# randyjhc/vit-colmap

Hardware: AMD Instinct MI355X
Metric: images/sec extracted + pair-matches/sec (N×D brute-force NN) (higher is better)
Workload: dtype bf16 (ViT) / u8+i32 (matcher); 1 GPU; configs[1]+configs[2]: DINOv2 ViT-S/14 extract of 50 640x480 images (512 keypoints, 384-D uint8 descriptors) then exhaustive mutual-NN + ratio matching of all pairs among the extracted images; images_total=50, images_rank0=50, num_keypoints=512, descriptor_dim=384, parallelism=images+pairs sharded x1

## Files before the change

vit_colmap_amd/csrc/attention.hip:

```cpp
#include <hip/hip_runtime.h>
#include <stdint.h>

#include "../../include/vitcolmap_hip.h"
#include "common.h"
#include "device.h"

namespace {

typedef __bf16 v8bf __attribute__((ext_vector_type(8)));
typedef __bf16 v4bf __attribute__((ext_vector_type(4)));
typedef __bf16 v2bf __attribute__((ext_vector_type(2)));
typedef short v4s __attribute__((ext_vector_type(4)));
typedef float v16f __attribute__((ext_vector_type(16)));

constexpr int kHD = 64;
constexpr int kWavesA = 4;
constexpr int kQW = 32;
constexpr int kQB = kWavesA * kQW;
constexpr int kKV = 64;
constexpr int kTileBytes = kKV * kHD * 2;

__device__ inline uint32_t k_off(int key, int slot) { return (uint32_t)key * 128u + (uint32_t)((slot ^ (key & 7)) << 4); }
__device__ inline uint32_t v_off(int key, int byte_in_row) {
  return (uint32_t)key * 128u + ((uint32_t)byte_in_row ^ (uint32_t)(((key >> 1) & 1) << 6));
}

constexpr float kLazyTh = 6.0f;
template <int QT, bool LAZY>
__global__ __launch_bounds__(256, (QT == 1 ? 3 : 2)) void attention_kernel(const __bf16* __restrict__ qkv,
                                                                           __bf16* __restrict__ out, int N, int H,
                                                                           float scale_log2e, int unit0, int nqb) {
  __shared__ __attribute__((aligned(16))) uint8_t lds[3][2][kTileBytes];
  const int tid = threadIdx.x, lane = tid & 63, wave = tid >> 6;
  const int r = lane & 31, hh = lane >> 5;
  const int unit = unit0 + (int)blockIdx.x;
  const int bh = unit / nqb, b = bh / H, h = bh - b * H;
  const int q_base = (unit - bh * nqb) * (kQB * QT);
  if (q_base >= N) return;
  const int q_row0 = q_base + wave * (kQW * QT) + r;
  const size_t tok_stride = (size_t)3 * H * kHD;
  const __bf16* base = qkv + (size_t)b * N * tok_stride + (size_t)h * kHD;

  v8bf qf[QT][4];
#pragma unroll
  for (int qt = 0; qt < QT; ++qt) {
    const __bf16* qp = base + (size_t)min(q_row0 + 32 * qt, N - 1) * tok_stride;
#pragma unroll
    for (int ks = 0; ks < 4; ++ks) qf[qt][ks] = *(const v8bf*)(qp + 16 * ks + 8 * hh);
  }
  __builtin_amdgcn_s_waitcnt(0x0F70);

  const int n_blk = (N + kKV - 1) / kKV;
  const uint32_t lds0 = vc::lds_addr(&lds[0][0][0]);
  const int wave_u = __builtin_amdgcn_readfirstlane(wave);
  uint32_t voff[4];
#pragma unroll
  for (int i = 0; i < 4; ++i) {
    const int pce = wave_u * 4 + i;
    const int which = pce >> 3, kg = pce & 7;
    const int krow = lane >> 3, cdst = lane & 7;
    const int key = kg * 8 + krow;
    const int csrc = which == 0 ? (cdst ^ krow) : (cdst ^ (((krow >> 1) & 1) << 2));
    voff[i] = (uint32_t)(((size_t)key * tok_stride + (size_t)(1 + which) * H * kHD + csrc * 8) * sizeof(__bf16));
  }
  const size_t blk_bytes = (size_t)kKV * tok_stride * sizeof(__bf16);
  auto issue_block = [&](int blk, int slot) {
    blk = min(blk, n_blk - 1);
    if ((blk + 1) * kKV <= N) {
      const char* sbase = (const char*)base + (size_t)blk * blk_bytes;
#pragma unroll
      for (int i = 0; i < 4; ++i) {
        const int pce = wave_u * 4 + i;
        const uint32_t dst = lds0 + (uint32_t)slot * (2 * kTileBytes) + (uint32_t)(pce >> 3) * kTileBytes + (uint32_t)(pce & 7) * 1024u;
        vc::lds_dma16(sbase, voff[i], dst);
      }
      return;
    }
#pragma unroll
    for (int i = 0; i < 4; ++i) {
      const int pce = wave_u * 4 + i;
      const int which = pce >> 3, kg = pce & 7;
      const int krow = lane >> 3, cdst = lane & 7;
      const int key = kg * 8 + krow;
      const int csrc = which == 0 ? (cdst ^ krow) : (cdst ^ (((krow >> 1) & 1) << 2));
      const int tok = min(blk * kKV + key, N - 1);
      const __bf16* src = base + (size_t)tok * tok_stride + (size_t)(1 + which) * H * kHD + csrc * 8;
      const uint32_t dst = lds0 + (uint32_t)slot * (2 * kTileBytes) + (uint32_t)which * kTileBytes + (uint32_t)kg * 1024u;
      vc::lds_dma16(src, dst);
    }
  };
  issue_block(0, 0);
  issue_block(1, 1);

  v16f acc_o[QT][2];
  float m_run[QT], l_run[QT];
#pragma unroll
  for (int qt = 0; qt < QT; ++qt) {
    m_run[qt] = -1e30f;
    l_run[qt] = 0.f;
#pragma unroll
    for (int dt = 0; dt < 2; ++dt)
#pragma unroll
      for (int i = 0; i < 16; ++i) acc_o[qt][dt][i] = 0.f;
  }

  const int grp = lane >> 4, gi = lane & 15, tq = gi >> 2, tp = gi & 3;

  int slot = 0;
  for (int blk = 0; blk < n_blk; ++blk) {
    asm volatile("s_waitcnt vmcnt(4)" ::: "memory");
    asm volatile("s_waitcnt lgkmcnt(0)\n\ts_barrier" ::: "memory");
    issue_block(blk + 2, slot == 0 ? 2 : slot - 1);
    const uint8_t* kt = lds[slot][0];
    const uint8_t* vt = lds[slot][1];

    v16f acc_s[QT][2];
#pragma unroll
    for (int qt = 0; qt < QT; ++qt) {
      float c0 = (LAZY && blk > 0) ? -m_run[qt] : 0.f;
      asm volatile("" : "+v"(c0));
#pragma unroll
      for (int t = 0; t < 2; ++t)
#pragma unroll
        for (int i = 0; i < 16; ++i) acc_s[qt][t][i] = c0;
    }
#pragma unroll
    for (int t = 0; t < 2; ++t) {
      const int key = t * 32 + r;
#pragma unroll
      for (int ks = 0; ks < 4; ++ks) {
        const v8bf kf = *(const v8bf*)(kt + k_off(key, 2 * ks + hh));
#pragma unroll
        for (int qt = 0; qt < QT; ++qt)
          acc_s[qt][t] = __builtin_amdgcn_mfma_f32_32x32x16_bf16(kf, qf[qt][ks], acc_s[qt][t], 0, 0, 0);
      }
    }
    if (blk == n_blk - 1 && (N & (kKV - 1)) != 0) {
      const int kv0 = blk * kKV;
#pragma unroll
      for (int qt = 0; qt < QT; ++qt)
#pragma unroll
        for (int t = 0; t < 2; ++t)
#pragma unroll
          for (int i = 0; i < 16; ++i) {
            const int key = kv0 + t * 32 + (i & 3) + 8 * (i >> 2) + 4 * hh;
            if (key >= N) acc_s[qt][t][i] = -1e30f;
          }
    }

    v8bf pf[QT][4];
#pragma unroll
    for (int qt = 0; qt < QT; ++qt) {
      if (LAZY && blk > 0) {
        int imax = __float_as_int(acc_s[qt][0][0]);
#pragma unroll
        for (int t = 0; t < 2; ++t)
#pragma unroll
          for (int i = 0; i < 16; ++i) imax = max(imax, __float_as_int(acc_s[qt][t][i]));
        if (!__any(imax > __float_as_int(kLazyTh))) {
          float lsum[4] = {0.f, 0.f, 0.f, 0.f};
#pragma unroll
          for (int s = 0; s < 4; ++s) {
            const int t = s >> 1, r0 = 8 * (s & 1);
#pragma unroll
            for (int j = 0; j < 8; ++j) {
              const float pj = __builtin_amdgcn_exp2f(acc_s[qt][t][r0 + j]);
              lsum[j & 3] += pj;
              pf[qt][s][j] = (__bf16)pj;
            }
          }
          l_run[qt] += (lsum[0] + lsum[1]) + (lsum[2] + lsum[3]);
          continue;
        }
#pragma unroll
        for (int t = 0; t < 2; ++t)
#pragma unroll
          for (int i = 0; i < 16; ++i) acc_s[qt][t][i] += m_run[qt];
      }
      float mloc = acc_s[qt][0][0];
#pragma unroll
      for (int t = 0; t < 2; ++t)
#pragma unroll
        for (int i = 0; i < 16; ++i) mloc = fmaxf(mloc, acc_s[qt][t][i]);
      mloc = fmaxf(mloc, __shfl_xor(mloc, 32));
      const float m_new = fmaxf(m_run[qt], mloc);
      if (!__all(m_new == m_run[qt])) {
        const float alpha = __builtin_amdgcn_exp2f((m_run[qt] - m_new) * scale_log2e);
        l_run[qt] *= alpha;
#pragma unroll
        for (int dt = 0; dt < 2; ++dt)
#pragma unroll
          for (int i = 0; i < 16; ++i) acc_o[qt][dt][i] *= alpha;
        m_run[qt] = m_new;
      }
      const float mb = m_run[qt] * scale_log2e;
      float lsum = 0.f;
#pragma unroll
      for (int s = 0; s < 4; ++s) {
        const int t = s >> 1, r0 = 8 * (s & 1);
#pragma unroll
        for (int j = 0; j < 8; ++j) {
          const float pj = __builtin_amdgcn_exp2f(__builtin_fmaf(acc_s[qt][t][r0 + j], scale_log2e, -mb));
          lsum += pj;
          pf[qt][s][j] = (__bf16)pj;
        }
      }
      l_run[qt] += lsum;
    }

#pragma unroll
    for (int dt = 0; dt < 2; ++dt) {
      const int dbase = 16 * (grp & 1) + 32 * dt;
#pragma unroll
      for (int s = 0; s < 4; ++s) {
        const int kbase = (s >> 1) * 32 + 16 * (s & 1) + 4 * hh;
        const int key0 = kbase + tq, key1 = kbase + 8 + tq;
        const v4s lo = __builtin_amdgcn_ds_read_tr16_b64_v4i16(
            (__attribute__((address_space(3))) v4s*)(vt + v_off(key0, (dbase + 4 * tp) * 2)));
        const v4s hi = __builtin_amdgcn_ds_read_tr16_b64_v4i16(
            (__attribute__((address_space(3))) v4s*)(vt + v_off(key1, (dbase + 4 * tp) * 2)));
        v8bf vf;
        *(v4s*)&vf = lo;
        *((v4s*)&vf + 1) = hi;
#pragma unroll
        for (int qt = 0; qt < QT; ++qt)
          acc_o[qt][dt] = __builtin_amdgcn_mfma_f32_32x32x16_bf16(vf, pf[qt][s], acc_o[qt][dt], 0, 0, 0);
      }
    }
    slot = slot == 2 ? 0 : slot + 1;
  }
  asm volatile("s_waitcnt vmcnt(0)" ::: "memory");

  typedef uint32_t v4u32a __attribute__((ext_vector_type(4)));
  __syncthreads();
  uint8_t* const stg = (uint8_t*)lds + wave * (QT * 4096);
  auto stg_at = [&](int row, int slot16) { return stg + row * 128 + ((slot16 ^ ((row >> 1) & 7)) << 4); };
#pragma unroll
  for (int qt = 0; qt < QT; ++qt) {
    const float l_tot = l_run[qt] + __shfl_xor(l_run[qt], 32);
    const float inv = 1.0f / l_tot;
#pragma unroll
    for (int dt = 0; dt < 2; ++dt) {
      uint32_t ep[8];
#pragma unroll
      for (int g4 = 0; g4 < 4; ++g4) {
        const v2bf lo = {(__bf16)(acc_o[qt][dt][4 * g4] * inv), (__bf16)(acc_o[qt][dt][4 * g4 + 1] * inv)};
        const v2bf hi = {(__bf16)(acc_o[qt][dt][4 * g4 + 2] * inv), (__bf16)(acc_o[qt][dt][4 * g4 + 3] * inv)};
        ep[2 * g4] = *(const uint32_t*)&lo;
        ep[2 * g4 + 1] = *(const uint32_t*)&hi;
      }
#pragma unroll
      for (int k = 0; k < 4; ++k) {
        const auto sw = __builtin_amdgcn_permlane32_swap(ep[k], ep[k + 4], false, false);
        ep[k] = sw[0];
        ep[k + 4] = sw[1];
      }
      const int row = 32 * qt + r;
      *(v4u32a*)stg_at(row, 4 * dt + 2 * hh) = (v4u32a){ep[0], ep[1], ep[4], ep[5]};
      *(v4u32a*)stg_at(row, 4 * dt + 2 * hh + 1) = (v4u32a){ep[2], ep[3], ep[6], ep[7]};
    }
  }
  {
    const int lrow = lane >> 3, lslot = lane & 7;
    const int q_wave0 = q_base + wave * (kQW * QT);
#pragma unroll
    for (int i = 0; i < 4 * QT; ++i) {
      const int row = 8 * i + lrow;
      const v4u32a o = *(const v4u32a*)stg_at(row, lslot);
      if (q_wave0 + row < N)
        *(v4u32a*)(out + ((size_t)b * N + q_wave0 + row) * (size_t)H * kHD + (size_t)h * kHD + lslot * 8) = o;
    }
  }
}

}

extern "C" {

int vc_attention_bf16(const void* qkv, int batch, int n_tokens, int n_heads, int head_dim, int q_prescaled, void* out,
                      vc_stream_t stream) {
  if (!qkv || !out || batch < 0 || n_tokens <= 0 || n_heads <= 0) return VC_ERR_INVALID_ARG;
  if (head_dim != kHD) return VC_ERR_UNSUPPORTED;
  if ((((uintptr_t)qkv) | ((uintptr_t)out)) % 16 != 0) return VC_ERR_INVALID_ARG;
  if (batch == 0) return VC_OK;
  const float scale_log2e = q_prescaled ? 1.0f : 0.125f * 1.4426950408889634f;
  const int qt = n_tokens >= 512 ? 2 : 1;
  const __bf16* pq = (const __bf16*)qkv;
  __bf16* po = (__bf16*)out;
  hipStream_t st = (hipStream_t)stream;
  const int bh = batch * n_heads;
#define VC_ATT(Q, L, UNITS, UNIT0, NQB) \
  hipLaunchKernelGGL((attention_kernel<Q, L>), dim3(UNITS), dim3(256), 0, st, pq, po, n_tokens, n_heads, scale_log2e, UNIT0, NQB)
  if (qt == 1) {
    const int nqb = (n_tokens + kQB - 1) / kQB;
    if (q_prescaled) VC_ATT(1, true, nqb * bh, 0, nqb); else VC_ATT(1, false, nqb * bh, 0, nqb);
    return vc::check_launch();
  }
  const int nqb2 = (n_tokens + 2 * kQB - 1) / (2 * kQB);
  if (q_prescaled) VC_ATT(2, true, nqb2 * bh, 0, nqb2); else VC_ATT(2, false, nqb2 * bh, 0, nqb2);
#undef VC_ATT
  return vc::check_launch();
}

}
```

Measured before the change: 7186 images/s.

## Speculatively skip lazy-rescale max check in attention, recompute on overflow

Wraps the flash-attention main loop in a templated pass. The lazy path first runs a fast pass that never computes the per-tile max check and never rescales, always exponentiating against the first block's running max. After the pass, a block-wide check on the row sum and output magnitude decides whether to redo the whole pass with the exact max-tracking path. This removes a per-tile reduction and a wave vote from the inner loop, at the cost of a full recomputation whenever scores exceed the first tile's max by enough to risk overflow or precision loss.

```diff
diff --git a/vit_colmap_amd/csrc/attention.hip b/vit_colmap_amd/csrc/attention.hip
--- a/vit_colmap_amd/csrc/attention.hip
+++ b/vit_colmap_amd/csrc/attention.hip
@@ -1,5 +1,7 @@
 #include <hip/hip_runtime.h>
 #include <stdint.h>
+
+#include <type_traits>
 
 #include "../../include/vitcolmap_hip.h"
 #include "common.h"
@@ -26,6 +28,7 @@
 }
 
 constexpr float kLazyTh = 6.0f;
+constexpr float kLMaxPerKey = 64.0f;
 template <int QT, bool LAZY>
 __global__ __launch_bounds__(256, (QT == 1 ? 3 : 2)) void attention_kernel(const __bf16* __restrict__ qkv,
                                                                            __bf16* __restrict__ out, int N, int H,
@@ -94,6 +97,11 @@
 
   v16f acc_o[QT][2];
   float m_run[QT], l_run[QT];
+
+  const int grp = lane >> 4, gi = lane & 15, tq = gi >> 2, tp = gi & 3;
+
+  auto run_pass = [&](auto fast_c) __attribute__((always_inline)) {
+  constexpr bool FAST = decltype(fast_c)::value;
 #pragma unroll
   for (int qt = 0; qt < QT; ++qt) {
     m_run[qt] = -1e30f;
@@ -103,9 +111,6 @@
 #pragma unroll
       for (int i = 0; i < 16; ++i) acc_o[qt][dt][i] = 0.f;
   }
-
-  const int grp = lane >> 4, gi = lane & 15, tq = gi >> 2, tp = gi & 3;
-
   int slot = 0;
   for (int blk = 0; blk < n_blk; ++blk) {
     asm volatile("s_waitcnt vmcnt(4)" ::: "memory");
@@ -152,12 +157,16 @@
 #pragma unroll
     for (int qt = 0; qt < QT; ++qt) {
       if (LAZY && blk > 0) {
-        int imax = __float_as_int(acc_s[qt][0][0]);
-#pragma unroll
-        for (int t = 0; t < 2; ++t)
-#pragma unroll
-          for (int i = 0; i < 16; ++i) imax = max(imax, __float_as_int(acc_s[qt][t][i]));
-        if (!__any(imax > __float_as_int(kLazyTh))) {
+        bool in_reach = true;
+        if constexpr (!FAST) {
+          int imax = __float_as_int(acc_s[qt][0][0]);
+#pragma unroll
+          for (int t = 0; t < 2; ++t)
+#pragma unroll
+            for (int i = 0; i < 16; ++i) imax = max(imax, __float_as_int(acc_s[qt][t][i]));
+          in_reach = !__any(imax > __float_as_int(kLazyTh));
+        }
+        if (in_reach) {
           float lsum[4] = {0.f, 0.f, 0.f, 0.f};
 #pragma unroll
           for (int s = 0; s < 4; ++s) {
@@ -230,6 +239,32 @@
     slot = slot == 2 ? 0 : slot + 1;
   }
   asm volatile("s_waitcnt vmcnt(0)" ::: "memory");
+  };
+
+  if constexpr (LAZY) {
+    run_pass(std::true_type{});
+    const float l_max = (float)N * kLMaxPerKey;
+    bool bad = false;
+#pragma unroll
+    for (int qt = 0; qt < QT; ++qt) {
+      const float l_tot = l_run[qt] + __shfl_xor(l_run[qt], 32);
+      const float inv = 1.0f / l_tot;
+      float oabs[4] = {0.f, 0.f, 0.f, 0.f};
+#pragma unroll
+      for (int dt = 0; dt < 2; ++dt)
+#pragma unroll
+        for (int i = 0; i < 16; ++i) oabs[i & 3] = __builtin_fmaf(__builtin_fabsf(acc_o[qt][dt][i]), inv, oabs[i & 3]);
+      const float osum = (oabs[0] + oabs[1]) + (oabs[2] + oabs[3]);
+      bad |= !(l_tot <= l_max) || !(osum <= 3.0e38f);
+    }
+    if (__syncthreads_or(bad)) {
+      issue_block(0, 0);
+      issue_block(1, 1);
+      run_pass(std::false_type{});
+    }
+  } else {
+    run_pass(std::false_type{});
+  }
 
   typedef uint32_t v4u32a __attribute__((ext_vector_type(4)));
   __syncthreads();
```

Result: faster. 7295 images/s (median of 6 runs) (+1.5%).
